# tomas-gr/RawNanoporeSignalCompression

Hardware: AMD Instinct MI355X
Metric: MSamples/s encode+decode (1/2/4/8 GPU) at fixed ratio; % HBM roofline (higher is better)
Workload: dtype int16; 1 GPU; configs[1]: 100000 reads x 100000 int16 samples per GPU (1 chunk each), C5 encode+decode; reads_per_gpu=100000, samples_per_read=100000, global_reads=100000, parallelism=dp1 (reads round-robin, no data-path collective)

## Files before the change

rawnanoporesignalcompression_amd/csrc/pgn_c5.h:

```cpp
#pragma once
#include "pgn_wave.h"

namespace pgn {

__device__ __forceinline__ uint16_t zz_enc16(uint16_t v) { return (uint16_t)((uint16_t)(v + v) ^ (uint16_t)((int16_t)v >> 15)); }
__device__ __forceinline__ uint16_t zz_dec16(uint16_t v) { return (uint16_t)((v >> 1) ^ (uint16_t)(0u - (v & 1u))); }

struct C5Streams {
    uint8_t *K, *S, *M, *Ll, *Lh;
};

constexpr uint32_t kSplitStep = 1024;
constexpr uint32_t kWinBytes = 1088;

struct SplitLds {
    alignas(16) uint8_t S[kWinBytes + 256];
    alignas(16) uint8_t M[kWinBytes + 256];
    alignas(16) uint8_t L[kWinBytes];
    alignas(16) uint8_t H[kWinBytes];
    alignas(16) uint32_t Z[64 * 8];
    alignas(16) uint8_t D[64 * 16];
};

typedef uint16_t pgn_u16x2 __attribute__((ext_vector_type(2)));
typedef int16_t pgn_s16x2 __attribute__((ext_vector_type(2)));
__device__ __forceinline__ pgn_u16x2 as_u16x2(uint32_t w) { return __builtin_bit_cast(pgn_u16x2, w); }
__device__ __forceinline__ uint32_t as_u32(pgn_u16x2 v) { return __builtin_bit_cast(uint32_t, v); }
__device__ __forceinline__ uint32_t pk_min_u16(uint32_t a, uint32_t b)
{
    uint32_t r;
    asm("v_pk_min_u16 %0, %1, %2" : "=v"(r) : "v"(a), "s"(b));
    return r;
}
__device__ __forceinline__ uint32_t pk_subsat_u16(uint32_t a, uint32_t b)
{
    uint32_t r;
    asm("v_pk_sub_u16 %0, %1, %2 clamp" : "=v"(r) : "v"(a), "s"(b));
    return r;
}
__device__ __forceinline__ uint32_t pk_sub_u16(uint32_t a, uint32_t b)
{
    uint32_t r;
    asm("v_pk_sub_u16 %0, %1, %2" : "=v"(r) : "v"(a), "v"(b));
    return r;
}

__device__ __forceinline__ uint32_t pack_nibbles(uint32_t w)
{
    const uint32_t y = w | (w >> 4);
    return (y & 0xFFu) | ((y >> 8) & 0xFF00u);
}

__device__ __forceinline__ void bwin_flush(uint8_t* W, uint32_t& fill, uint8_t* out, uint32_t& gpos)
{
    const uint32_t lane = (uint32_t)lane_id();
    const uint32_t nblk = fill >> 4, tail = fill & 15u;
    for (uint32_t b = lane; b < nblk; b += 64) gst<uint4>(out + gpos + 16u * b, *(const uint4*)(W + 16u * b));
    if (nblk) {
        const uint8_t v = W[16u * nblk + (lane & 15u)];
        if (lane < tail) W[lane] = v;
    }
    gpos += 16u * nblk;
    fill = tail;
}

__device__ __forceinline__ void nwin_flush(uint8_t* W, uint32_t& fill, uint8_t* out, uint32_t& gpos)
{
    const uint32_t lane = (uint32_t)lane_id();
    const uint32_t nblk = fill >> 5, tail = fill & 31u;
    for (uint32_t b = lane; b < nblk; b += 64) {
        const uint4 a = *(const uint4*)(W + 32u * b), c = *(const uint4*)(W + 32u * b + 16u);
        uint4 o;
        o.x = pack_nibbles(a.x) | (pack_nibbles(a.y) << 16);
        o.y = pack_nibbles(a.z) | (pack_nibbles(a.w) << 16);
        o.z = pack_nibbles(c.x) | (pack_nibbles(c.y) << 16);
        o.w = pack_nibbles(c.z) | (pack_nibbles(c.w) << 16);
        gst<uint4>(out + gpos + 16u * b, o);
    }
    if (nblk) {
        const uint8_t v = W[32u * nblk + (lane & 31u)];
        if (lane < tail) W[lane] = v;
    }
    gpos += 16u * nblk;
    fill = tail;
}

template <bool C4> struct ClassOffsets {
    static constexpr uint32_t o1 = C4 ? 0u : 1u, o2 = C4 ? 0u : 17u, o3 = C4 ? 0u : 273u;
    static constexpr uint32_t t1 = C4 ? 15u : 16u, t2 = C4 ? 255u : 272u;
};

__device__ __forceinline__ uint32_t bfi32(uint32_t m, uint32_t a, uint32_t b)
{
    uint32_t r;
    asm("v_bfi_b32 %0, %1, %2, %3" : "=v"(r) : "v"(m), "v"(a), "v"(b));
    return r;
}

template <bool Full, bool C4 = false>
__device__ __forceinline__ uint32_t split_step(const uint4& a, const uint4& b, const int16_t* __restrict__ x, uint32_t n,
                                               uint32_t t, SplitLds& W, uint32_t& fS, uint32_t& fM, uint32_t& fL,
                                               uint32_t& prevX)
{
    using CO = ClassOffsets<C4>;
    const uint32_t lane = (uint32_t)lane_id();
    const uint32_t i0 = t + 16u * lane;
    uint32_t wd[8];
    if (Full) {
        wd[0] = a.x; wd[1] = a.y; wd[2] = a.z; wd[3] = a.w;
        wd[4] = b.x; wd[5] = b.y; wd[6] = b.z; wd[7] = b.w;
    } else {
#pragma unroll
        for (int k = 0; k < 8; k++) {
            const uint32_t lo = (i0 + 2u * k < n) ? (uint32_t)gld<uint16_t>(x + i0 + 2 * k) : 0u;
            const uint32_t hi = (i0 + 2u * k + 1u < n) ? (uint32_t)gld<uint16_t>(x + i0 + 2 * k + 1) : 0u;
            wd[k] = lo | (hi << 16);
        }
    }
    uint32_t prv = dpp<kDppWaveShr1>(wd[7] >> 16);
    prv = (lane == 0) ? prevX : prv;
    prevX = readlane_u32(wd[7] >> 16, 63);
    constexpr uint32_t kOne = 0x00010001u, kT1 = CO::t1 * kOne, kT2 = CO::t2 * kOne;
    uint32_t z[8], val[8], cp[8], c2[8], c3[8];
#pragma unroll
    for (int k = 0; k < 8; k++) {
        const uint32_t before = (k == 0) ? ((wd[0] << 16) | prv) : __builtin_amdgcn_alignbit(wd[k], wd[k - 1], 16);
        const pgn_u16x2 d = as_u16x2(wd[k]) - as_u16x2(before);
        z[k] = as_u32((d << (pgn_u16x2){1, 1}) ^ __builtin_bit_cast(pgn_u16x2, __builtin_bit_cast(pgn_s16x2, d) >> (pgn_s16x2){15, 15}));
    }
#pragma unroll
    for (int k = 0; k < 8; k++) c2[k] = pk_subsat_u16(z[k], kT1);
#pragma unroll
    for (int k = 0; k < 8; k++) c3[k] = pk_subsat_u16(z[k], kT2);
#pragma unroll
    for (int k = 0; k < 8; k++) cp[k] = pk_min_u16(z[k], kOne);
#pragma unroll
    for (int k = 0; k < 8; k++) c2[k] = pk_min_u16(c2[k], kOne);
#pragma unroll
    for (int k = 0; k < 8; k++) c3[k] = pk_min_u16(c3[k], kOne);
#pragma unroll
    for (int k = 0; k < 8; k++) {
        cp[k] += c2[k] + c3[k];
        if (!Full) {
            const uint32_t vm = ((i0 + 2u * k < n) ? 0xFFFFu : 0u) | ((i0 + 2u * k + 1u < n) ? 0xFFFF0000u : 0u);
            cp[k] &= vm;
        }
    }
#pragma unroll
    for (int k = 0; k < 8; k++) val[k] = C4 ? z[k] : pk_sub_u16(z[k], kOne + (c2[k] << 4));
    const uint32_t X = cp[0] | (cp[1] << 4) | (cp[2] << 8) | (cp[3] << 12);
    const uint32_t Y = cp[4] | (cp[5] << 4) | (cp[6] << 8) | (cp[7] << 12);
    const uint32_t Xn = (X & 0x3333u) | ((X >> 14) & 0xCCCCu), Yn = (Y & 0x3333u) | ((Y >> 14) & 0xCCCCu);
    const uint32_t kw = Xn | (Yn << 16);
    const uint32_t lo = kw & 0x55555555u, hi = (kw >> 1) & 0x55555555u;
    const uint32_t m1 = lo & ~hi, m2 = hi & ~lo, m3 = lo & hi;
    const uint32_t pc = (uint32_t)__builtin_popcount(m1) | ((uint32_t)__builtin_popcount(m2) << 11) |
                        ((uint32_t)__builtin_popcount(m3) << 22);
    const uint32_t inc = wave_incl_sum(pc);
    const uint32_t tot = readlane_u32(inc, 63);
    const uint32_t exc = inc - pc;
    uint8_t* const wb = reinterpret_cast<uint8_t*>(&W);
    constexpr uint32_t offS = (uint32_t)__builtin_offsetof(SplitLds, S), offM = (uint32_t)__builtin_offsetof(SplitLds, M);
    const uint32_t baseS = offS + fS + (exc & 0x7FFu), baseM = offM + fM + ((exc >> 11) & 0x7FFu);
    constexpr uint32_t offD = (uint32_t)__builtin_offsetof(SplitLds, D);
    static_assert(sizeof(SplitLds) < 65536, "split places are 16-bit");
    const uint32_t dD = offD + 16u * lane;
    uint32_t plo = dD | (baseS << 16), phi = baseM | (dD << 16);
#pragma unroll
    for (int m = 0; m < 16; m++) {
        const uint32_t c = __builtin_amdgcn_ubfe(kw, 2 * m, 2);
        const uint32_t at = __builtin_amdgcn_perm(phi, plo, c * 0x0202u + 0x0C0C0100u);
        if (m < 15) {
            const uint64_t inc = (uint64_t)1 << (16 * c);
            plo += (uint32_t)inc;
            phi += (uint32_t)(inc >> 32);
        }
        wb[at] = (uint8_t)(val[m >> 1] >> (16 * (m & 1)));
    }
    const uint32_t t3 = (readlane_u32(exc, 63) >> 22) + (readlane_u32(pc, 63) >> 22);
    if (t3) {
        if (m3) {
#pragma unroll
            for (int k = 0; k < 8; k++) W.Z[8 * lane + k] = z[k];
            uint32_t qL = fL + (exc >> 22);
            const uint16_t* zs = reinterpret_cast<const uint16_t*>(W.Z) + 16 * lane;
            for (uint32_t mm = m3; mm; mm &= mm - 1u) {
                const uint32_t w = (uint32_t)zs[__builtin_ctz(mm) >> 1] - CO::o3;
                W.L[qL] = (uint8_t)w;
                W.H[qL] = (uint8_t)(w >> 8);
                qL++;
            }
        }
    }
    fS += tot & 0x7FFu;
    fM += (tot >> 11) & 0x7FFu;
    fL += t3;
    return kw;
}

template <bool C4 = false>
__device__ __forceinline__ void c5_split_wave(const int16_t* __restrict__ x, uint32_t n, const C5Streams& st, uint32_t sizes[5],
                                              SplitLds& W)
{
    const uint32_t lane = (uint32_t)lane_id();
    uint32_t fS = 0, fM = 0, fL = 0, fH = 0;
    uint32_t gS = 0, gM = 0, gL = 0, gH = 0;
    uint32_t prevX = 0;
    uint4 na = make_uint4(0u, 0u, 0u, 0u), nb = na;
    auto ld16 = [&](const int16_t* p) { return gld<uint4>(p); };
    if (kSplitStep <= n) {
        na = ld16(x + 16u * lane);
        nb = ld16(x + 16u * lane + 8);
    }
    for (uint32_t t = 0; t < n; t += kSplitStep) {
        const bool full = t + kSplitStep <= n;
        const uint4 ca = na, cb = nb;
        if (t + 2 * kSplitStep <= n) {
            na = ld16(x + t + kSplitStep + 16u * lane);
            nb = ld16(x + t + kSplitStep + 16u * lane + 8);
        }
        const uint32_t kw = full ? split_step<true, C4>(ca, cb, x, n, t, W, fS, fM, fL, prevX)
                                 : split_step<false, C4>(ca, cb, x, n, t, W, fS, fM, fL, prevX);
        fH = fL;
        const uint32_t nK = full ? kSplitStep / 4 : (n - t + 3) / 4;
        uint8_t* kout = st.K + (t >> 2);
        if (4u * lane + 4u <= nK) gst<uint32_t>(kout + 4u * lane, kw);
        else for (uint32_t b = 4u * lane; b < nK; b++) gst<uint8_t>(kout + b, (uint8_t)(kw >> (8u * (b - 4u * lane))));
        lds_sync();
        nwin_flush(W.S, fS, st.S, gS);
        bwin_flush(W.M, fM, st.M, gM);
        bwin_flush(W.L, fL, st.Ll, gL);
        bwin_flush(W.H, fH, st.Lh, gH);
        lds_sync();
    }
    const uint32_t nbS = (fS + 1) / 2;
    for (uint32_t j = lane; j < nbS; j += 64) {
        const uint32_t lo = W.S[2 * j], hi = (2 * j + 1 < fS) ? W.S[2 * j + 1] : 0u;
        gst<uint8_t>(st.S + gS + j, (uint8_t)(lo | (hi << 4)));
    }
    for (uint32_t j = lane; j < fM; j += 64) gst<uint8_t>(st.M + gM + j, W.M[j]);
    for (uint32_t j = lane; j < fL; j += 64) {
        gst<uint8_t>(st.Ll + gL + j, W.L[j]);
        gst<uint8_t>(st.Lh + gH + j, W.H[j]);
    }
    lds_sync();
    sizes[0] = (n + 3) / 4;
    sizes[1] = gS + nbS;
    sizes[2] = gM + fM;
    sizes[3] = gL + fL;
    sizes[4] = gL + fL;
}

__device__ __forceinline__ void bwin_flush_lead(uint8_t* W, uint32_t& fill, uint8_t* out, uint32_t& gpos, uint32_t& lead)
{
    const uint32_t lane = (uint32_t)lane_id();
    const uint32_t nblk = fill >> 4, tail = fill & 15u;
    for (uint32_t b = lane; b < nblk; b += 64) {
        if (b == 0 && lead) {
            for (uint32_t k = lead; k < 16; k++) gst<uint8_t>(out + gpos + k, W[k]);
        } else {
            gst<uint4>(out + gpos + 16u * b, *(const uint4*)(W + 16u * b));
        }
    }
    if (nblk) {
        const uint8_t v = W[16u * nblk + (lane & 15u)];
        if (lane < tail) W[lane] = v;
        lead = 0;
    }
    gpos += 16u * nblk;
    fill = tail;
}
__device__ __forceinline__ void nwin_flush_lead(uint8_t* W, uint32_t& fill, uint8_t* out, uint32_t& gpos, uint32_t& lead)
{
    const uint32_t lane = (uint32_t)lane_id();
    const uint32_t nblk = fill >> 5, tail = fill & 31u;
    for (uint32_t b = lane; b < nblk; b += 64) {
        if (b == 0 && lead) {
            for (uint32_t k = (lead + 1) >> 1; k < 16; k++) gst<uint8_t>(out + gpos + k, (uint8_t)(W[2 * k] | (W[2 * k + 1] << 4)));
        } else {
            const uint4 a = *(const uint4*)(W + 32u * b), c = *(const uint4*)(W + 32u * b + 16u);
            uint4 o;
            o.x = pack_nibbles(a.x) | (pack_nibbles(a.y) << 16);
            o.y = pack_nibbles(a.z) | (pack_nibbles(a.w) << 16);
            o.z = pack_nibbles(c.x) | (pack_nibbles(c.y) << 16);
            o.w = pack_nibbles(c.z) | (pack_nibbles(c.w) << 16);
            gst<uint4>(out + gpos + 16u * b, o);
        }
    }
    if (nblk) {
        const uint8_t v = W[32u * nblk + (lane & 31u)];
        if (lane < tail) W[lane] = v;
        lead = 0;
    }
    gpos += 16u * nblk;
    fill = tail;
}

template <bool C4 = false>
__device__ inline void c5_split_range(const int16_t* __restrict__ x, uint32_t n, uint32_t t0, uint32_t t1,
                                      const C5Streams& st, uint32_t pS, uint32_t pM, uint32_t pL, SplitLds& W,
                                      uint32_t& firstNib, uint32_t& lastNib)
{
    const uint32_t lane = (uint32_t)lane_id();
    uint32_t fS = pS & 31u, fM = pM & 15u, fL = pL & 15u, fH = fL;
    uint32_t gS = (pS >> 1) & ~15u, gM = pM & ~15u, gL = pL & ~15u, gH = gL;
    uint32_t leadS = fS, leadM = fM, leadL = fL, leadH = fL;
    uint32_t prevX = t0 ? (uint32_t)(uint16_t)__builtin_amdgcn_readfirstlane((int)gld<uint16_t>(x + t0 - 1)) : 0u;
    firstNib = 0xFFu;
    lastNib = 0xFFu;
    uint4 na = make_uint4(0u, 0u, 0u, 0u), nb = na;
    if (t0 + kSplitStep <= n) {
        na = gld<uint4>(x + t0 + 16u * lane);
        nb = gld<uint4>(x + t0 + 16u * lane + 8);
    }
    for (uint32_t t = t0; t < t1; t += kSplitStep) {
        const bool full = t + kSplitStep <= n;
        const uint4 ca = na, cb = nb;
        if (t + kSplitStep < t1 && t + 2 * kSplitStep <= n) {
            na = gld<uint4>(x + t + kSplitStep + 16u * lane);
            nb = gld<uint4>(x + t + kSplitStep + 16u * lane + 8);
        }
        const uint32_t kw = full ? split_step<true, C4>(ca, cb, x, n, t, W, fS, fM, fL, prevX)
                                 : split_step<false, C4>(ca, cb, x, n, t, W, fS, fM, fL, prevX);
        fH = fL;
        const uint32_t nK = full ? kSplitStep / 4 : (n - t + 3) / 4;
        uint8_t* kout = st.K + (t >> 2);
        if (4u * lane + 4u <= nK) gst<uint32_t>(kout + 4u * lane, kw);
        else for (uint32_t b = 4u * lane; b < nK; b++) gst<uint8_t>(kout + b, (uint8_t)(kw >> (8u * (b - 4u * lane))));
        lds_sync();
        if (firstNib == 0xFFu && (pS & 1u) && fS > leadS) firstNib = W.S[leadS];
        nwin_flush_lead(W.S, fS, st.S, gS, leadS);
        bwin_flush_lead(W.M, fM, st.M, gM, leadM);
        bwin_flush_lead(W.L, fL, st.Ll, gL, leadL);
        bwin_flush_lead(W.H, fH, st.Lh, gH, leadH);
        lds_sync();
    }
    const uint32_t nbS = (fS + 1) / 2;
    for (uint32_t j = lane; j < nbS; j += 64) {
        if (2 * j < leadS || 2 * j + 1 >= fS) continue;
        gst<uint8_t>(st.S + gS + j, (uint8_t)(W.S[2 * j] | (W.S[2 * j + 1] << 4)));
    }
    if (fS > leadS && (fS & 1u)) lastNib = W.S[fS - 1];
    for (uint32_t j = leadM + lane; j < fM; j += 64) gst<uint8_t>(st.M + gM + j, W.M[j]);
    for (uint32_t j = leadL + lane; j < fL; j += 64) {
        gst<uint8_t>(st.Ll + gL + j, W.L[j]);
        gst<uint8_t>(st.Lh + gH + j, W.H[j]);
    }
    lds_sync();
}

template <bool C4 = false>
__device__ inline void c5_split_counts(const int16_t* __restrict__ x, uint32_t n, uint32_t t0, uint32_t t1, uint32_t& cS,
                                       uint32_t& cM, uint32_t& cL)
{
    using CO = ClassOffsets<C4>;
    const uint32_t lane = (uint32_t)lane_id();
    uint32_t s = 0, m = 0, l = 0;
    for (uint32_t tb = t0; tb < t1; tb += 4096u) {
        uint32_t wv[4][8], pv[4];
#pragma unroll
        for (int u = 0; u < 4; u++) {
            const uint32_t t = tb + 1024u * u + 16u * lane;
            pv[u] = (t < t1 && t) ? (uint32_t)gld<uint16_t>(x + t - 1) : 0u;
            if (t + 16u <= t1) {
                const uint4 a = gld<uint4>(x + t), b = gld<uint4>(x + t + 8);
                wv[u][0] = a.x; wv[u][1] = a.y; wv[u][2] = a.z; wv[u][3] = a.w;
                wv[u][4] = b.x; wv[u][5] = b.y; wv[u][6] = b.z; wv[u][7] = b.w;
            } else {
#pragma unroll
                for (uint32_t k = 0; k < 8; k++) {
                    const uint32_t lo = t + 2 * k < t1 ? (uint32_t)gld<uint16_t>(x + t + 2 * k) : 0u;
                    const uint32_t hi = t + 2 * k + 1 < t1 ? (uint32_t)gld<uint16_t>(x + t + 2 * k + 1) : 0u;
                    wv[u][k] = lo | (hi << 16);
                }
            }
        }
#pragma unroll
// ... 437 lines not shown
```

rawnanoporesignalcompression_amd/csrc/pgn_zenc.h:

```cpp
#pragma once
#ifndef PGN_AB_SKIP
#define PGN_AB_SKIP 0
#endif
#include "pgn_c5.h"
#include "pgn_wave.h"
#include "zstd1_model.h"

namespace pgn {

constexpr int kWinWords = 392;
constexpr int kFiltSlots = 512;

struct WCTable {
    uint32_t tableLog;
    uint16_t stateTable[64];
    uint32_t deltaNbBits[16];
    int32_t deltaFindState[16];
};

struct alignas(16) EncLds {
    union {
        struct {
            uint64_t filt[kFiltSlots];
            uint32_t vh0[64], vh1[64], vpk[64];
// ... 406 lines not shown
                    if (isC0) c0 = false;
                    else c1 = false;
                }
                hits = ballot(rep || c0 || c1);
            }
        }
        const uint64_t vmask = ballot(valid);
        const int f = hits ? __builtin_ctzll(hits) : 64;
        const int lastCommit = hits ? f : (63 - __builtin_clzll(vmask));
        if (valid && (int)lane <= lastCommit) {
            const uint64_t upto = (lastCommit >= 63) ? ~0ull : ((1ull << (lastCommit + 1)) - 1ull);
            bool w0 = (h0 != h1), w1 = true;
            for (uint64_t cand = M0 & above & upto; cand && w0;) {
                const int jj = __builtin_ctzll(cand);
                if (L.vh0[jj] == h0 || L.vh1[jj] == h0) w0 = false;
                cand &= cand - 1;
            }
            for (uint64_t cand = M1 & above & upto; cand && w1;) {
                const int jj = __builtin_ctzll(cand);
                if (L.vh0[jj] == h1 || L.vh1[jj] == h1) w1 = false;
                cand &= cand - 1;
            }
            if (w0) gst<uint32_t>(ht + h0, (tag << kTagShift) | fp0 | ((uint32_t)pk + 1));
            if (w1) gst<uint32_t>(ht + h1, (tag << kTagShift) | fp1 | ((uint32_t)pk + 2));
        }
        lds_sync();
        if (!hits) {
            wave_sync();
            if (vmask == ~0ull) {
                ip0 = pNext;
                ci += 64;
                pk = pkN;
                pNext = pNextN;
                v8 = v8N;
                repw = repwN;
                havePk = true;
                continue;
            }
            break;
        }
        const int32_t ipf = (int32_t)L.vpk[f];
        const bool repf = (ballot(rep) >> f) & 1, c0f = (ballot(c0) >> f) & 1;
        const uint32_t m0f = readlane_u32(m0, f), m1f = readlane_u32(m1, f);
        const uint32_t cur0 = (uint32_t)ipf + 1;
        int32_t ipm, match0;
        uint32_t mLength, offcode;
        if (repf) {
            const int32_t ip2 = ipf + 2;
            mLength = (gb(src + (ip2 - 1)) == gb(src + (ip2 - (int32_t)off1 - 1))) ? 1u : 0u;
            ipm = ip2 - (int32_t)mLength;
            match0 = ipm - (int32_t)off1;
            mLength += 4;
            offcode = 0;
        } else {
            if (c0f) { ipm = ipf; match0 = (int32_t)m0f - 1; }
            else { ipm = ipf + 1; match0 = (int32_t)m1f - 1; }
            off2 = off1;
            off1 = (uint32_t)(ipm - match0);
            offcode = off1 + 2;
            mLength = 4;
            const int32_t room = match0 - ((int32_t)lowIdx - 1);
            const int32_t lim = (ipm - anchor) < room ? (ipm - anchor) : room;
            const uint32_t back = lim > 0 ? wave_back_count(src, (uint32_t)ipm, (uint32_t)match0, (uint32_t)lim) : 0u;
            ipm -= (int32_t)back;
            match0 -= (int32_t)back;
            mLength += back;
        }
        mLength += fwdKnown ? fwdKnown - 4u
                            : wave_match_count(src, (uint32_t)ipm + mLength, (uint32_t)match0 + mLength, (uint32_t)iend);
        if (lane == 0) {
            seqs[nbSeq].litLength = (uint32_t)(ipm - anchor);
            seqs[nbSeq].offset = offcode + 1;
            seqs[nbSeq].mlBase = mLength - 3;
        }
        nbSeq++;
        ip0 = ipm + (int32_t)mLength;
        anchor = ip0;
        chain = 0;
        ci = 0;
        if (ip0 <= ilimit) {
            uint64_t wa = 0, wb = 0;
            if (lane == 0) {
                wa = ld64u(src + cur0 + 1);
                wb = ld64u(src + ip0 - 2);
            }
            uint32_t rc0 = 0, rc1 = 0;
            if (off2 > 0) {
                rc0 = ld32u(src + ip0);
                rc1 = ld32u(src + ip0 - (int32_t)off2);
            }
            positions(0, pk, pNext);
            loads(pk, v8, repw);
            havePk = true;
            if (lane == 0) {
                gst<uint32_t>(ht + z1::hash_word(wa, hlog, mls), ht_entry(tag, cur0 + 2, (uint32_t)wa, idxBits));
                gst<uint32_t>(ht + z1::hash_word(wb, hlog, mls), ht_entry(tag, (uint32_t)(ip0 - 2) + 1, (uint32_t)wb, idxBits));
            }
            if (off2 > 0) {
                bool firstRep = true;
                while ((ip0 <= ilimit) &&
                       (firstRep ? rc0 == rc1 : ld32u(src + ip0) == ld32u(src + ip0 - (int32_t)off2))) {
                    firstRep = false;
                    havePk = false;
                    const uint32_t rLength = wave_match_count(src, (uint32_t)ip0 + 4, (uint32_t)ip0 + 4 - off2, (uint32_t)iend) + 4;
                    const uint32_t t = off2;
                    off2 = off1;
                    off1 = t;
                    if (lane == 0) {
                        const uint64_t wr = ld64u(src + ip0);
                        gst<uint32_t>(ht + z1::hash_word(wr, hlog, mls), ht_entry(tag, (uint32_t)ip0 + 1, (uint32_t)wr, idxBits));
                        seqs[nbSeq].litLength = 0;
                        seqs[nbSeq].offset = 1;
                        seqs[nbSeq].mlBase = rLength - 3;
                    }
                    nbSeq++;
                    ip0 += (int32_t)rLength;
                    anchor = ip0;
                }
            }
        }
        wave_sync();
    }
    SearchOut r;
    r.nbSeq = nbSeq;
    r.lastLL = (uint32_t)(iend - anchor);
    r.rep0 = off1 ? off1 : offSaved;
    r.rep1 = off2 ? off2 : offSaved;
    r.rounds = rounds;
    r.candIters = candIters;
    return r;
}

__device__ __noinline__ void huf_encode_segment_wave(uint8_t* __restrict__ out, const uint8_t* __restrict__ src, uint32_t len,
                                                     uint32_t totalBits, lds_u32* win)
{
    const uint32_t lane = (uint32_t)lane_id();
    out = uni(out);
    src = uni(src);
    len = uni(len);
    totalBits = uni(totalBits);
    const uint32_t* cw = sEnc.cw;
    for (uint32_t w = lane; w < (uint32_t)kWinWords; w += 64) win[w] = 0;
    lds_sync();
    uint32_t winLo = 0;
    uint32_t bitBase = 0;
    uint4 nv = make_uint4(0, 0, 0, 0);
    if ((int32_t)len - 16 - (int32_t)(16 * lane) >= 0) nv = gld<uint4>(src + (len - 16 - 16 * lane));
    auto step = [&](auto FULL, uint32_t r0) {
        const int32_t a = (int32_t)len - 16 - (int32_t)(r0 + 16 * lane);
        uint32_t wv[4];
        if (FULL || a >= 0) {
            const uint4 v = nv;
            wv[0] = v.x; wv[1] = v.y; wv[2] = v.z; wv[3] = v.w;
            if (a - 1024 >= 0) nv = gld<uint4>(src + (a - 1024));
        } else {
#pragma unroll
            for (int q = 0; q < 4; q++) {
                uint32_t x = 0;
#pragma unroll
                for (int b = 0; b < 4; b++) {
                    const int32_t i = a + 4 * q + b;
                    if (i >= 0) x |= (uint32_t)gb(src + i) << (8 * b);
                }
                wv[q] = x;
            }
        }
        const int32_t nvalid = (int32_t)len - (int32_t)(r0 + 16 * lane);
        uint64_t grp[4];
        uint32_t gnb[4];
        uint32_t myBits = 0;
#pragma unroll
        for (int g = 0; g < 4; g++) {
            uint64_t acc = 0;
            uint32_t n = 0;
#pragma unroll
            for (int jj = 0; jj < 4; jj++) {
                const int j = 4 * g + jj;
                const uint32_t sym = (wv[(15 - j) >> 2] >> (8 * ((15 - j) & 3))) & 0xFFu;
                uint32_t cwj = cw[sym];
                if (!FULL) cwj = (j < nvalid) ? cwj : 0u;
                acc |= (uint64_t)(cwj & 0xFFFFu) << n;
                n += cwj >> 16;
            }
            grp[g] = acc;
            gnb[g] = n;
            myBits += n;
        }
        const uint32_t incl = wave_incl_sum(myBits);
        const uint32_t stepBits = readlane_u32(incl, 63);
        uint32_t pos = bitBase + (incl - myBits) - winLo;
#pragma unroll
        for (int g = 0; g < 4; g++) {
            const uint32_t w = pos >> 5, sh = pos & 31;
            const uint64_t lo = grp[g] << sh;
            __hip_atomic_fetch_or(&win[w], (uint32_t)lo, __ATOMIC_RELAXED, __HIP_MEMORY_SCOPE_WAVEFRONT);
            __hip_atomic_fetch_or(&win[w + 1], (uint32_t)(lo >> 32), __ATOMIC_RELAXED, __HIP_MEMORY_SCOPE_WAVEFRONT);
            __hip_atomic_fetch_or(&win[w + 2], (uint32_t)((grp[g] >> 32) >> (32 - sh)), __ATOMIC_RELAXED,
                                  __HIP_MEMORY_SCOPE_WAVEFRONT);
            pos += gnb[g];
        }
        lds_sync();
        const uint32_t endRel = bitBase + stepBits - winLo;
        const uint32_t complete = endRel >> 5;
        uint8_t* o = out + (winLo >> 3);
        const uint32_t carry = win[complete];
        for (uint32_t w = lane; w <= complete; w += 64) {
            const uint32_t v = win[w];
            if (w < complete) __builtin_nontemporal_store(v, (__attribute__((address_space(1))) uint32_t*)(o + 4 * w));
            win[w] = 0u;
        }
        if (lane == 0) win[0] = carry;
        lds_sync();
        winLo += complete * 32;
        bitBase += stepBits;
    };
    uint32_t r0 = 0;
    for (; r0 + 1024 <= len; r0 += 1024) step(std::true_type{}, r0);
    if (r0 < len) step(std::false_type{}, r0);
    if (lane == 0) {
        const uint32_t rel = totalBits - winLo;
        win[rel >> 5] |= 1u << (rel & 31);
    }
    lds_sync();
    const uint32_t nbytes = ((totalBits + 8) >> 3) - (winLo >> 3);
    uint8_t* o = out + (winLo >> 3);
    for (uint32_t b = lane; b < nbytes; b += 64) gst<uint8_t>(o + b, (uint8_t)(win[b >> 2] >> (8 * (b & 3))));
    lds_sync();
}

constexpr int kCoopEncWaves = 4;
struct CoopEncCmd {
    uint32_t op;
    uint32_t n, segSize;
    const uint8_t* lit;
    uint8_t* out[4];
    uint32_t bits[4];
};
typedef __attribute__((address_space(3))) CoopEncCmd lds_enc_cmd;

__device__ __noinline__ void hist_segment_wave(const uint8_t* __restrict__ lit, uint32_t n, uint32_t segSize, uint32_t k)
{
    EncLds& L = sEnc;
    const uint32_t lane = (uint32_t)lane_id();
    lit = uni(lit);
    n = uni(n);
    segSize = uni(segSize);
    k = uni(k);
    const uint32_t a0 = k * segSize, a1 = (k + 1) * segSize < n ? (k + 1) * segSize : n;
    uint32_t* h = &L.hist2[k >> 1][0];
    const uint32_t inc = 1u << (16 * (k & 1));
    for (uint32_t i0 = a0 + 16u * lane; i0 < a1; i0 += 4096) {
        uint4 v[4];
#pragma unroll
        for (int u = 0; u < 4; u++) {
            const uint32_t i = i0 + 1024u * (uint32_t)u;
            if (i + 16 <= a1) {
                v[u] = gld<uint4>(lit + i);
            } else {
                uint32_t w[4] = {0, 0, 0, 0};
                for (uint32_t b = 0; b < 16; b++)
                    if (i + b < a1) w[b >> 2] |= (uint32_t)gb(lit + i + b) << (8 * (b & 3));
                v[u] = make_uint4(w[0], w[1], w[2], w[3]);
            }
        }
#pragma unroll
        for (int u = 0; u < 4; u++) {
            const uint32_t i = i0 + 1024u * (uint32_t)u;
            const uint32_t wd[4] = {v[u].x, v[u].y, v[u].z, v[u].w};
            if (i + 16 <= a1) {
#pragma unroll
                for (int b = 0; b < 16; b++) atomicAdd(h + ((wd[b >> 2] >> (8 * (b & 3))) & 0xFFu), inc);
            } else {
                for (uint32_t b = 0; b < 16; b++)
                    if (i + b < a1) atomicAdd(h + ((wd[b >> 2] >> (8 * (b & 3))) & 0xFFu), inc);
            }
        }
    }
}

__device__ __noinline__ void coop_enc_helper_wave(uint32_t wid, lds_enc_cmd* cmd, lds_u32* win)
{
    while (true) {
        __syncthreads();
        const uint32_t op = cmd->op;
        if (op == 0) break;
        if (op == 1) hist_segment_wave(cmd->lit, cmd->n, cmd->segSize, wid);
        else {
            const uint32_t a = cmd->segSize * wid, e = wid == 3 ? cmd->n : a + cmd->segSize;
            huf_encode_segment_wave(cmd->out[wid], cmd->lit + a, e - a, cmd->bits[wid], win);
        }
        __syncthreads();
    }
}
__device__ __forceinline__ void coop_enc_finish(lds_enc_cmd* cmd)
{
    if (lane_id() == 0) cmd->op = 0;
    __syncthreads();
}

__device__ __noinline__ uint32_t huf_tree_wave(uint32_t maxSym, uint32_t maxNbBits, uint32_t nnz, PhaseProf& P)
{
    EncLds& L = sEnc;
    const int lane = lane_id();
    maxSym = uni(maxSym);
    maxNbBits = uni(maxNbBits);
    nnz = uni(nnz);
    z1::HufNode* hn = L.nodes + 1;
    constexpr int kStart = z1::kHufStartNode;
    const int nonNullRank = (int)nnz - 1;
    const int nodeRoot = kStart + nonNullRank - 1;
    P.count(2);
    L.nodes[0].count = 1u << 31;
    uint32_t* pickVal = L.count;
    int lowS = nonNullRank, lowN = kStart, nodeNb = kStart;
    uint32_t rounds = 0;
    while (nodeNb <= nodeRoot) {
        rounds++;
        uint32_t s;
        {
            const uint32_t S0 = lowS >= 0 ? hn[lowS].count : (1u << 31);
            const uint32_t S1 = lowS >= 1 ? hn[lowS - 1].count : (1u << 31);
            const uint32_t Q0 = lowN < nodeNb ? hn[lowN].count : (1u << 30);
            const uint32_t Q1 = lowN + 1 < nodeNb ? hn[lowN + 1].count : (1u << 30);
            s = (S0 < Q0) ? S0 + (S1 < Q0 ? S1 : Q0) : Q0 + (S0 < Q1 ? S0 : Q1);
        }
        const uint32_t nq = (uint32_t)(nodeNb - lowN);
        const int leafSlots = (lowS + 64) >> 6;
        uint32_t nl = 0;
        uint32_t lv[4];
#pragma unroll
        for (int j = 0; j < 4; j++) {
            lv[j] = 0xFFFFFFFFu;
            if (j < leafSlots) {
                const int i = lane + 64 * j;
                if (i <= lowS) lv[j] = hn[lowS - i].count;
                nl += (uint32_t)__builtin_popcountll(ballot(lv[j] < s));
            }
        }
        nl = uni(nl);
        const uint32_t t = nl + nq, pairs = t >> 1, used = 2 * pairs;
        uint32_t usedLeaves = 0;
        const uint32_t stN = nq ? (1u << (31 - __builtin_clz(nq))) : 0u;
#pragma unroll
        for (int j = 0; j < 4; j++) {
            if (j < leafSlots) {
                const uint32_t i = (uint32_t)lane + 64u * (uint32_t)j;
                uint32_t lo = 0;
                for (uint32_t st = stN; st; st >>= 1) {
                    const uint32_t k = lo + st, kc = k < nq ? k : nq;
                    lo = hn[lowN + (int)kc - 1].count <= lv[j] ? kc : lo;
                }
                const uint32_t pos = i + lo;
                const bool take = i < nl && pos < used;
                if (take) {
                    hn[lowS - (int)i].parent = (uint16_t)(nodeNb + (int)(pos >> 1));
                    pickVal[pos] = lv[j];
                }
// ... 1022 lines not shown
            uint32_t cwq;
            if (useOld) cwq = gld<uint32_t>(prevCw + s);
            else cwq = ((uint32_t)s <= maxSym) ? ((uint32_t)L.val[s] | ((uint32_t)L.nbBits[s] << 16)) : 0u;
            L.cw[s] = cwq;
            const uint32_t nbq = cwq >> 16;
#pragma unroll
            for (int k = 0; k < 4; k++) b4[k] += seg_count(L, k, s) * nbq;
        }
#pragma unroll
        for (int k = 0; k < 4; k++) {
            bits[k] = wave_sum(b4[k]);
            bytes[k] = (bits[k] + 8) >> 3;
        }
    }
    uint32_t cStreams = single ? bytes[0] : 6 + bytes[0] + bytes[1] + bytes[2] + bytes[3];
    uint32_t total = hSize + cStreams;
    if (total >= n - 1 || total >= n - minGain) { size_t r = write_raw_literals_wave(dst, lit, n); P.mark(7); return ret(r, false); }
    if (lhSize + total >= rawAt) { P.mark(7); return ret(lhSize + total, false); }
    if (!useOld && saveNew) {
#pragma unroll
        for (int q = 0; q < 4; q++) gst<uint32_t>(nextCw + lane + 64 * q, L.cw[lane + 64 * q]);
    }
    if (lane == 0) {
        z1::write_huf_lit_header(dst, lhSize, n, total, single, useOld ? z1::kSetRepeat : z1::kSetCompressed);
        if (!single) {
            z1::wr16(dst + lhSize + hSize, bytes[0]);
            z1::wr16(dst + lhSize + hSize + 2, bytes[1]);
            z1::wr16(dst + lhSize + hSize + 4, bytes[2]);
        }
    }
    for (uint32_t i = (uint32_t)lane; i < hSize; i += 64) gst<uint8_t>(dst + lhSize + i, L.hdr[i]);
    wave_sync();
    uint8_t* op = dst + lhSize + hSize + (single ? 0 : 6);
    if (COOP && !single) {
        if (lane == 0) {
            coop->op = 2;
            coop->lit = lit;
            coop->n = n;
            coop->segSize = segSize;
            uint8_t* o = op;
            for (int k = 0; k < 4; k++) {
                coop->out[k] = o;
                coop->bits[k] = bits[k];
                o += bytes[k];
            }
        }
        __syncthreads();
        huf_encode_segment_wave(op, lit, segSize, bits[0], (lds_u32*)sEnc.win);
        __syncthreads();
    } else {
        for (int k = 0; k < nseg; k++) {
            uint32_t a = segSize * (uint32_t)k;
            uint32_t e = (k == nseg - 1) ? n : a + segSize;
#if PGN_AB_SKIP != 4
            huf_encode_segment_wave(op, lit + a, e - a, bits[k], (lds_u32*)sEnc.win);
#endif
            P.count(7, (e - a + 1023) / 1024);
            op += bytes[k];
        }
    }
    P.mark(6);
    return ret(lhSize + total, !useOld);
}

__device__ inline bool wave_is_rle(const uint8_t* p, uint32_t n)
{
    const uint8_t b0 = gb(p);
    bool diff = false;
    for (uint32_t i = (uint32_t)lane_id(); i < n; i += 64) diff |= gb(p + i) != b0;
    return !ballot(diff);
}

template <bool COOP = false>
__device__ __noinline__ size_t zstd1_compress_wave(uint8_t* __restrict__ dst, const uint8_t* __restrict__ src, uint32_t n,
                                             EncScratch S, uint32_t tag, PhaseProf& P)
{
    dst = uni(dst);
    src = uni(src);
    n = uni(n);
    tag = uni(tag);
    S.ht = uni(S.ht);
    S.seqs = uni(S.seqs);
    S.codes = uni(S.codes);
    S.lit = uni(S.lit);
    S.seqSection = uni(S.seqSection);
    S.seqWork = uni(S.seqWork);
    S.maxSeq = uni(S.maxSeq);
    S.huf = uni(S.huf);
    const int lane = lane_id();
    if (n == 0) {
        if (lane == 0) z1::write_empty_frame(dst);
        return 9;
    }
    const size_t h = z1::frame_header_size(n, n < 7 ? 10u : z1::level1_params(n).windowLog);
    if (n < 7) {
        if (lane == 0) z1::write_raw_block_frame(dst, src, n);
        return h + 3 + n;
    }
    const z1::Params p = z1::level1_params(n);
    P.count(12);
    if (lane == 0) z1::write_frame_header(dst, n, p.windowLog);
    size_t o = h;
    uint32_t rep0 = 1, rep1 = 4;
    uint32_t hufCur = 0, hufCheck = 0;
    for (uint32_t start = 0; start < n; start += (uint32_t)z1::kMaxSrc) {
        const uint32_t bs = (n - start < (uint32_t)z1::kMaxSrc) ? n - start : (uint32_t)z1::kMaxSrc;
        const bool last = start + bs == n, first = start == 0;
        uint8_t* bdst = dst + o;
        uint32_t cSize = 0;
        size_t seqSize = 0;
#if PGN_AB_SKIP == 1
        if (false) {
#else
        if (bs >= 7) {
#endif
            const uint32_t ip0 = start + (start == 0 ? 1u : 0u);
            const SearchOut so = fast_search_wave(src, start, start + bs, p.hashLog, p.mls, S.ht, tag, S.seqs, rep0, rep1,
                                                  ht_idx_bits(n), z1::window_low_index(start + bs, p.windowLog),
                                                  ip0 + 1u - z1::window_low_index(ip0, p.windowLog), first && last);
            const uint32_t nbSeq = uni(so.nbSeq), lastLL = uni(so.lastLL);
            P.mark(1);
            P.count(0, uni(so.rounds));
            P.count(14, uni(so.candIters));
            P.count(1, nbSeq);
            P.count(13);
#if PGN_AB_SKIP == 2
            if (uni(so.nbSeq) < 0x7FFFFFFFu) goto raw_block;
#endif
            const uint8_t* lit = src + start;
            uint32_t nLit = bs;
            if (nbSeq > 0) {
                uint32_t pos = start, q = 0;
                for (uint32_t i = 0; i < nbSeq; i++) {
                    const z1::Seq sq = S.seqs[i];
                    wave_copy(S.lit + q, src + pos, sq.litLength);
                    q += sq.litLength;
                    pos += sq.litLength + sq.mlBase + 3;
                }
                wave_copy(S.lit + q, src + pos, lastLL);
                q += lastLL;
                wave_sync();
                lit = S.lit;
                nLit = q;
                P.mark(2);
            }
            uint8_t* body = bdst + 3;
            const uint32_t maxCSize = bs - ((bs >> 6) + 2);
            const LitOut lo = compress_literals_wave<COOP>(body, lit, nLit, P, nbSeq > 0 ? 1u : 0u, S.huf + 256 * hufCur,
                                                           hufCheck, S.huf + 256 * (hufCur ^ 1u), last ? 0u : 1u,
                                                           nbSeq == 0 ? maxCSize - 1u : 0xFFFFFFFFu, S.coop);
            const size_t litSize = uni(lo.size);
            wave_sync();
            if (nbSeq == 0) {
                if (lane == 0) body[litSize] = 0;
                seqSize = 1;
            } else {
                P.count(10);
                P.count(11, nbSeq);
                const size_t r = seq_section_wave(S, nbSeq);
                seqSize = (r == (size_t)-1 || r == (size_t)-2) ? (size_t)-1 : r;
                P.mark(8);
            }
            if (seqSize != (size_t)-1 && litSize + seqSize < maxCSize) cSize = (uint32_t)(litSize + seqSize);
            if (!first && cSize < 25 && wave_is_rle(src + start, bs)) cSize = 1;
            if (cSize > 1) {
                rep0 = uni(so.rep0);
                rep1 = uni(so.rep1);
                if (uni(lo.newTable)) {
                    hufCur ^= 1u;
                    hufCheck = 1;
                }
            }
        }
#if PGN_AB_SKIP == 2
    raw_block:
#endif
        wave_sync();
        size_t bsz;
        if (cSize == 0) {
            if (lane == 0) z1::wr24(bdst, (uint32_t)((last ? 1u : 0u) + (z1::kBtRaw << 1) + (bs << 3)));
            wave_copy_nt(bdst + 3, src + start, bs);
            bsz = 3 + bs;
        } else if (cSize == 1) {
            if (lane == 0) {
                z1::wr24(bdst, (uint32_t)((last ? 1u : 0u) + (z1::kBtRle << 1) + (bs << 3)));
                bdst[3] = src[start];
            }
            bsz = 4;
        } else {
            if (seqSize > 1) wave_copy(bdst + 3 + (cSize - seqSize), S.seqSection, seqSize);
            if (lane == 0) z1::wr24(bdst, (uint32_t)((last ? 1u : 0u) + (z1::kBtCompressed << 1) + (cSize << 3)));
            bsz = 3 + cSize;
        }
        o += bsz;
        wave_sync();
        P.mark(9);
    }
    return o;
}

}
```

Measured before the change: 234,300 MSamples/s.

## Make full-step stream flushes branch-free with fixed-shape clamped vector stores

The C5 split loop now handles full 1024-sample steps separately from the tail. The S and M window flushes use fixed per-lane 16-byte stores with clamped indices, which can write duplicate bytes, and L/H flushes run only when there is enough data. The next-input prefetch is made unconditional by clamping its address. The zstd bitstream writer's full steps now flush whole 16-byte groups with vector stores instead of per-word nontemporal stores, at the cost of extra LDS barriers. Redundant overlapping stores and a pre-zeroing of the output heads are added, along with a bounds guard on the zero byte written after the literals.

```diff
diff --git a/rawnanoporesignalcompression_amd/csrc/pgn_c5.h b/rawnanoporesignalcompression_amd/csrc/pgn_c5.h
--- a/rawnanoporesignalcompression_amd/csrc/pgn_c5.h
+++ b/rawnanoporesignalcompression_amd/csrc/pgn_c5.h
@@ -77,6 +77,39 @@
         o.w = pack_nibbles(c.z) | (pack_nibbles(c.w) << 16);
         gst<uint4>(out + gpos + 16u * b, o);
     }
+    if (nblk) {
+        const uint8_t v = W[32u * nblk + (lane & 31u)];
+        if (lane < tail) W[lane] = v;
+    }
+    gpos += 16u * nblk;
+    fill = tail;
+}
+
+__device__ __forceinline__ void bwin_flush_fixed(uint8_t* W, uint32_t& fill, uint8_t* out, uint32_t& gpos)
+{
+    const uint32_t lane = (uint32_t)lane_id();
+    const uint32_t nblk = fill >> 4, tail = fill & 15u;
+    const uint32_t b = lane < nblk ? lane : nblk;
+    gst<uint4>(out + gpos + 16u * b, *(const uint4*)(W + 16u * b));
+    if (nblk) {
+        const uint8_t v = W[16u * nblk + (lane & 15u)];
+        if (lane < tail) W[lane] = v;
+    }
+    gpos += 16u * nblk;
+    fill = tail;
+}
+__device__ __forceinline__ void nwin_flush_fixed(uint8_t* W, uint32_t& fill, uint8_t* out, uint32_t& gpos)
+{
+    const uint32_t lane = (uint32_t)lane_id();
+    const uint32_t nblk = fill >> 5, tail = fill & 31u;
+    const uint32_t b = lane < nblk ? lane : nblk;
+    const uint4 a = *(const uint4*)(W + 32u * b), c = *(const uint4*)(W + 32u * b + 16u);
+    uint4 o;
+    o.x = pack_nibbles(a.x) | (pack_nibbles(a.y) << 16);
+    o.y = pack_nibbles(a.z) | (pack_nibbles(a.w) << 16);
+    o.z = pack_nibbles(c.x) | (pack_nibbles(c.y) << 16);
+    o.w = pack_nibbles(c.z) | (pack_nibbles(c.w) << 16);
+    gst<uint4>(out + gpos + 16u * b, o);
     if (nblk) {
         const uint8_t v = W[32u * nblk + (lane & 31u)];
         if (lane < tail) W[lane] = v;
@@ -208,21 +241,37 @@
     uint32_t prevX = 0;
     uint4 na = make_uint4(0u, 0u, 0u, 0u), nb = na;
     auto ld16 = [&](const int16_t* p) { return gld<uint4>(p); };
-    if (kSplitStep <= n) {
+    const uint32_t nfull = n & ~(kSplitStep - 1u);
+    if (nfull) {
         na = ld16(x + 16u * lane);
         nb = ld16(x + 16u * lane + 8);
-    }
-    for (uint32_t t = 0; t < n; t += kSplitStep) {
-        const bool full = t + kSplitStep <= n;
+        gst<uint32_t>(st.K + 4u * lane, 0u);
+        gst<uint4>(st.S, make_uint4(0u, 0u, 0u, 0u));
+        gst<uint4>(st.M, make_uint4(0u, 0u, 0u, 0u));
+    }
+    uint32_t t = 0;
+    for (; t < nfull; t += kSplitStep) {
         const uint4 ca = na, cb = nb;
-        if (t + 2 * kSplitStep <= n) {
-            na = ld16(x + t + kSplitStep + 16u * lane);
-            nb = ld16(x + t + kSplitStep + 16u * lane + 8);
-        }
-        const uint32_t kw = full ? split_step<true, C4>(ca, cb, x, n, t, W, fS, fM, fL, prevX)
-                                 : split_step<false, C4>(ca, cb, x, n, t, W, fS, fM, fL, prevX);
+        const uint32_t tn = t + 2 * kSplitStep <= n ? t + kSplitStep : t;
+        na = ld16(x + tn + 16u * lane);
+        nb = ld16(x + tn + 16u * lane + 8);
+        const uint32_t kw = split_step<true, C4>(ca, cb, x, n, t, W, fS, fM, fL, prevX);
         fH = fL;
-        const uint32_t nK = full ? kSplitStep / 4 : (n - t + 3) / 4;
+        lds_sync();
+        if (fL >= 16) {
+            bwin_flush(W.L, fL, st.Ll, gL);
+            bwin_flush(W.H, fH, st.Lh, gH);
+        }
+        gst<uint32_t>(st.K + (t >> 2) + 4u * lane, kw);
+        nwin_flush_fixed(W.S, fS, st.S, gS);
+        bwin_flush_fixed(W.M, fM, st.M, gM);
+        lds_sync();
+    }
+    if (t < n) {
+        const uint4 ca = na, cb = nb;
+        const uint32_t kw = split_step<false, C4>(ca, cb, x, n, t, W, fS, fM, fL, prevX);
+        fH = fL;
+        const uint32_t nK = (n - t + 3) / 4;
         uint8_t* kout = st.K + (t >> 2);
         if (4u * lane + 4u <= nK) gst<uint32_t>(kout + 4u * lane, kw);
         else for (uint32_t b = 4u * lane; b < nK; b++) gst<uint8_t>(kout + b, (uint8_t)(kw >> (8u * (b - 4u * lane))));
diff --git a/rawnanoporesignalcompression_amd/csrc/pgn_zenc.h b/rawnanoporesignalcompression_amd/csrc/pgn_zenc.h
--- a/rawnanoporesignalcompression_amd/csrc/pgn_zenc.h
+++ b/rawnanoporesignalcompression_amd/csrc/pgn_zenc.h
@@ -582,7 +582,8 @@
         if (FULL || a >= 0) {
             const uint4 v = nv;
             wv[0] = v.x; wv[1] = v.y; wv[2] = v.z; wv[3] = v.w;
-            if (a - 1024 >= 0) nv = gld<uint4>(src + (a - 1024));
+            if (FULL) nv = gld<uint4>(src + (a - 1024 >= 0 ? a - 1024 : 0));
+            else if (a - 1024 >= 0) nv = gld<uint4>(src + (a - 1024));
         } else {
 #pragma unroll
             for (int q = 0; q < 4; q++) {
@@ -633,6 +634,23 @@
         const uint32_t endRel = bitBase + stepBits - winLo;
         const uint32_t complete = endRel >> 5;
         uint8_t* o = out + (winLo >> 3);
+        if (FULL) {
+            const uint32_t nq = complete >> 2, last = nq ? nq - 1u : 0u;
+            const uint32_t keep = lane < 4 ? win[4 * nq + lane] : 0u;
+            const uint32_t q0 = lane < last ? lane : last, q1 = lane + 64 < last ? lane + 64 : last;
+            const uint4 v0 = make_uint4(win[4 * q0], win[4 * q0 + 1], win[4 * q0 + 2], win[4 * q0 + 3]);
+            const uint4 v1 = make_uint4(win[4 * q1], win[4 * q1 + 1], win[4 * q1 + 2], win[4 * q1 + 3]);
+            gst<uint4>(o + 16 * q0, v0);
+            gst<uint4>(o + 16 * q1, v1);
+            lds_sync();
+            for (uint32_t w = lane; w <= complete; w += 64) win[w] = 0u;
+            lds_sync();
+            if (lane < 4) win[lane] = keep;
+            lds_sync();
+            winLo += nq * 128;
+            bitBase += stepBits;
+            return;
+        }
         const uint32_t carry = win[complete];
         for (uint32_t w = lane; w <= complete; w += 64) {
             const uint32_t v = win[w];
@@ -1961,7 +1979,7 @@
             const size_t litSize = uni(lo.size);
             wave_sync();
             if (nbSeq == 0) {
-                if (lane == 0) body[litSize] = 0;
+                if (lane == 0 && litSize + 1 < maxCSize) body[litSize] = 0;
                 seqSize = 1;
             } else {
                 P.count(10);
```

New measurement: 240,000 MSamples/s, median of 6. 2.4% higher.
